# Daniel-Starr/pointcloudhookup

Hardware: AMD Instinct MI355X
Metric: Mpts/s ground-filter+tower-cluster, 100 M-pt corridor; % HBM roofline on kNN (higher is better)
Workload: dtype f32 (filter) + f64 (distance predicate)

## Files before the change

### pointcloudhookup_amd/csrc/pch_dbscan.hip

```cpp
#include "pch_prims.h"

namespace pch {

constexpr int DB_THREADS = 256;
constexpr int DB_WAVES   = DB_THREADS / 64;
constexpr int DB_ROWS    = 25;
constexpr int INT_BIG    = 0x7fffffff;
constexpr int DB_FEW_QUERIES = 24;
constexpr int DB_AHEAD = 3;
constexpr long long DB_LONG_TOT = 8192;
constexpr int DB_SEGS = 43;

struct DbGrid {
    float   ox, oy, oz;
    double  cell;
    double  inv_cell;
    double  eps2;
    float   eps2_lo, eps2_hi;
    int     bx, by, bz;
    int     mx, my, mz;
    int64_t chunk_size;
    const uint32_t* chunk_bad;
    const uint32_t* chunk_cells;
    int     min_samples;
};

__constant__ int8_t DB_ROW_DY[DB_ROWS] = {0, 1, -1, 0, 0, 1, 1, -1, -1, 2, -2, 0, 0,
                                          2, 2, -2, -2, 1, 1, -1, -1, 2, 2, -2, -2};
__constant__ int8_t DB_ROW_DZ[DB_ROWS] = {0, 0, 0, 1, -1, 1, -1, 1, -1, 0, 0, 2, -2,
                                          1, -1, 1, -1, 2, -2, 2, -2, 2, -2, 2, -2};

__device__ __forceinline__ uint64_t db_pack(const DbGrid& g, uint64_t chunk, uint64_t cz,
                                            uint64_t cy, uint64_t cx) {
    return ((((chunk << g.bz) | cz) << g.by | cy) << g.bx) | cx;
}

__device__ __forceinline__ bool db_within(const float4& q, const float4& p, double eps2) {
    const double dx = (double)q.x - (double)p.x;
    const double dy = (double)q.y - (double)p.y;
    const double dz = (double)q.z - (double)p.z;
    double d = dx * dx;
    d += dy * dy;
    d += dz * dz;
    return d <= eps2;
}

__device__ __forceinline__ bool db_within2(const float4& q, const float4& p, const DbGrid& g) {
    const float dx = q.x - p.x, dy = q.y - p.y, dz = q.z - p.z;
    float d = dx * dx;
    d = __builtin_fmaf(dy, dy, d);
    d = __builtin_fmaf(dz, dz, d);
    if (d <= g.eps2_lo) return true;
    if (d >= g.eps2_hi) return false;
    return db_within(q, p, g.eps2);
}

typedef float f32x2 __attribute__((ext_vector_type(2)));
struct __attribute__((aligned(16))) DbPair { f32x2 x, y, z, pad; };

__device__ __forceinline__ void db_tile_put(DbPair* __restrict__ tile, int l, const float4& p) {
    float* f = reinterpret_cast<float*>(&tile[l >> 1]);
    f[l & 1] = p.x; f[2 + (l & 1)] = p.y; f[4 + (l & 1)] = p.z;
}
__device__ __forceinline__ float4 db_tile_get(const DbPair* __restrict__ tile, int k) {
    const float* f = reinterpret_cast<const float*>(&tile[k >> 1]);
    float4 p;
    p.x = f[k & 1]; p.y = f[2 + (k & 1)]; p.z = f[4 + (k & 1)]; p.w = 0.0f;
    return p;
}
__device__ __forceinline__ int db_tile_count(const float4& q, const DbPair* __restrict__ tile, int nj,
                                             const DbGrid& g) {
    const f32x2 qx = {q.x, q.x}, qy = {q.y, q.y}, qz = {q.z, q.z};
    const float lo = g.eps2_lo, hi = g.eps2_hi;
    int c_lo = 0, c_hi = 0;
    const int np = ((nj + 7) & ~7) >> 1;
    for (int k = 0; k < np; k += 4) {
        f32x2 px[4], py[4], pz[4];
#pragma unroll
        for (int u = 0; u < 4; ++u) { px[u] = tile[k + u].x; py[u] = tile[k + u].y; pz[u] = tile[k + u].z; }
#pragma unroll
        for (int u = 0; u < 4; ++u) {
            const f32x2 dx = qx - px[u], dy = qy - py[u], dz = qz - pz[u];
            f32x2 d = dx * dx;
            d = __builtin_elementwise_fma(dy, dy, d);
            d = __builtin_elementwise_fma(dz, dz, d);
            c_lo += (d.x <= lo ? 1 : 0) + (d.y <= lo ? 1 : 0);
            c_hi += (d.x < hi ? 1 : 0) + (d.y < hi ? 1 : 0);
        }
    }
    if (c_lo != c_hi) {
        c_lo = 0;
        for (int k = 0; k < nj; ++k) c_lo += db_within2(q, db_tile_get(tile, k), g) ? 1 : 0;
    }
// ... 638 lines not shown
            cell_key[cc[j]] = key;
            uint4* a4 = reinterpret_cast<uint4*>(cell_acc + 8 * (int64_t)cc[j]);
            a4[0] = make_uint4(0u, 0u, 0u, 0u);
            a4[1] = make_uint4(0u, 0u, 0u, 0u);
            const uint64_t ch = sh < 64 ? key >> sh : 0, pch = sh < 64 ? pk >> sh : 0;
            if (i == 0 || ch != pch) chunk_cells[ch] = cc[j];
        }
        if (i == n - 1) { cell_start[cc[j] + 1] = (uint32_t)n; chunk_cells[nchunks] = cc[j] + 1; }
    }
    if (base + DC_ITEMS <= n) {
        uint4* o = reinterpret_cast<uint4*>(cid + base);
        o[0] = make_uint4(cc[0], cc[1], cc[2], cc[3]);
        o[1] = make_uint4(cc[4], cc[5], cc[6], cc[7]);
    } else {
#pragma unroll
        for (int j = 0; j < DC_ITEMS; ++j)
            if (base + j < n) cid[base + j] = cc[j];
    }
}
struct RowSet {
    int ca[DB_ROWS], cb[DB_ROWS];
};

__device__ __forceinline__ int db_lower(const uint64_t* __restrict__ a, int m, uint64_t k) {
    int lo = 0, hi = m;
    while (lo < hi) { const int mid = (lo + hi) >> 1; if (a[mid] < k) lo = mid + 1; else hi = mid; }
    return lo;
}
__device__ __forceinline__ int2 db_row_run(const DbGrid& g, const uint64_t* __restrict__ cell_key, uint64_t key,
                                           int row) {
    const uint64_t cx = key & ((1ull << g.bx) - 1);
    const uint64_t cy = (key >> g.bx) & ((1ull << g.by) - 1);
    const uint64_t cz = (key >> (g.bx + g.by)) & ((1ull << g.bz) - 1);
    const int sh = g.bx + g.by + g.bz;
    const uint64_t chunk = sh < 64 ? (key >> sh) : 0;
    const int ny = (int)cy + DB_ROW_DY[row], nz = (int)cz + DB_ROW_DZ[row];
    int2 v;
    v.x = 0; v.y = 0;
    if (ny >= 0 && ny <= g.my && nz >= 0 && nz <= g.mz) {
        const int xlo = (int)cx - 2 < 0 ? 0 : (int)cx - 2;
        const int xhi = (int)cx + 2 > g.mx ? g.mx : (int)cx + 2;
        const int c0 = (int)g.chunk_cells[chunk], c1 = (int)g.chunk_cells[chunk + 1];
        v.x = c0 + db_lower(cell_key + c0, c1 - c0, db_pack(g, chunk, (uint64_t)nz, (uint64_t)ny, (uint64_t)xlo));
        const uint64_t khi = db_pack(g, chunk, (uint64_t)nz, (uint64_t)ny, (uint64_t)xhi);
        uint64_t kk[5];
#pragma unroll
        for (int i = 0; i < 5; ++i) kk[i] = v.x + i < c1 ? cell_key[v.x + i] : ~0ull;
        int cntx = 0;
#pragma unroll
        for (int i = 0; i < 5; ++i) cntx += kk[i] <= khi ? 1 : 0;
        v.y = v.x + cntx;
    }
    return v;
}

__device__ __forceinline__ void db_rows(const DbGrid& g, const uint64_t* __restrict__ cell_key, uint64_t key,
                                        RowSet* __restrict__ rs, const int2* __restrict__ rowtab, int cell) {
    const int l = lane_id();
    if (rowtab) {
        if (l < DB_ROWS) {
            const int2 v = rowtab[(int64_t)cell * DB_ROWS + l];
            rs->ca[l] = v.x;
            rs->cb[l] = v.y;
        }
        __builtin_amdgcn_wave_barrier();
        return;
    }
    if (l < DB_ROWS) {
        const int2 v = db_row_run(g, cell_key, key, l);
        rs->ca[l] = v.x;
        rs->cb[l] = v.y;
    }
    __builtin_amdgcn_wave_barrier();
}

__global__ __launch_bounds__(DB_THREADS) void db_rowtab_k(DbGrid g, const uint64_t* __restrict__ cell_key,
                                                          int m, int2* __restrict__ rowtab) {
    const int c = (blockIdx.x * DB_WAVES + wave_id()) * 2 + (lane_id() >> 5);
    const int l = lane_id() & 31;
    if (c >= m || l >= DB_ROWS) return;
    rowtab[(int64_t)c * DB_ROWS + l] = db_row_run(g, cell_key, cell_key[c], l);
}

template <bool COUNT>
__global__ __launch_bounds__(DB_THREADS) void db_core_k(DbGrid g, const float4* __restrict__ pts,
                                                        const uint32_t* __restrict__ cell_start,
                                                        const uint64_t* __restrict__ cell_key, int m,
                                                        const int2* __restrict__ rowtab,
                                                        uint8_t* __restrict__ core_s,
                                                        uint32_t* __restrict__ cell_ncore,
                                                        unsigned long long* __restrict__ stats) {
    unsigned long long n_useful = 0, n_slots = 0, n_tiles = 0;
    auto tally = [&]() {
        if (COUNT && lane_id() == 0) {
            atomicAdd(&stats[0], n_useful); atomicAdd(&stats[1], n_slots);
            atomicAdd(&stats[2], 1ull); atomicAdd(&stats[3], n_tiles);
        }
    };
    __shared__ RowSet rows[DB_WAVES];
    __shared__ DbPair tiles[DB_WAVES][32];
    __shared__ uint32_t seg_a[DB_WAVES][DB_SEGS], seg_b[DB_WAVES][DB_SEGS];
    const int c = blockIdx.x * DB_WAVES + wave_id();
    if (c >= m) return;
    const int l = lane_id();
    const uint32_t s = cell_start[c], e = cell_start[c + 1];
    const int cnt = (int)(e - s);
    {
        const int sh = g.bx + g.by + g.bz;
        if (g.chunk_bad[sh < 64 ? (cell_key[c] >> sh) : 0]) {
            for (uint32_t i = s + l; i < e; i += 64) core_s[i] = 0;
            if (l == 0) cell_ncore[c] = 0;
            return;
        }
    }
    if (cnt >= g.min_samples) {
        for (uint32_t i = s + l; i < e; i += 64) core_s[i] = 1;
        if (l == 0) cell_ncore[c] = (uint32_t)cnt;
        return;
    }
    RowSet* rs = &rows[wave_id()];
    db_rows(g, cell_key, cell_key[c], rs, rowtab, c);
    long long tot = 0;
    if (l < DB_ROWS) tot = (long long)cell_start[rs->cb[l]] - (long long)cell_start[rs->ca[l]];
    tot = wave_reduce_add(tot);
    if (tot < (long long)g.min_samples) {
        for (uint32_t i = s + l; i < e; i += 64) core_s[i] = 0;
        if (l == 0) cell_ncore[c] = 0;
        return;
    }
    uint32_t* sa = seg_a[wave_id()];
    uint32_t* sb = seg_b[wave_id()];
    {
        const uint64_t xmask = (1ull << g.bx) - 1;
        const int cx = (int)(cell_key[c] & xmask);
        if (l < DB_ROWS) {
            const int ca = rs->ca[l], cb = rs->cb[l];
            if (l < 9) {
                int ia = ca, ib = cb;
                if (ca < cb) {
                    if ((int)(cell_key[ca] & xmask) == cx - 2) ia = ca + 1;
                    if (ib > ia && (int)(cell_key[cb - 1] & xmask) == cx + 2) ib = cb - 1;
                }
                sa[l] = cell_start[ia];      sb[l] = cell_start[ib];
                sa[9 + l] = cell_start[ca];  sb[9 + l] = cell_start[ia];
                sa[18 + l] = cell_start[ib]; sb[18 + l] = cell_start[cb];
            } else {
                sa[18 + l] = cell_start[ca]; sb[18 + l] = cell_start[cb];
            }
        }
        __builtin_amdgcn_wave_barrier();
    }
    uint32_t ncore = 0;
    const bool long_sweep = tot >= DB_LONG_TOT;
    if (cnt < DB_FEW_QUERIES) {
        for (uint32_t q = s; q < e; ++q) {
            const float4 qp = pts[q];
            int count = 0;
            if (long_sweep) {
                for (int r = 0; r < DB_SEGS && count < g.min_samples; ++r) {
                    const uint32_t pa = sa[r], pb = sb[r];
                    for (uint32_t j0 = pa; j0 < pb && count < g.min_samples; j0 += 64u * DB_AHEAD) {
                        float4 P[DB_AHEAD];
#pragma unroll
                        for (int u = 0; u < DB_AHEAD; ++u) {
                            const uint32_t j = j0 + 64u * u + l;
                            P[u] = pts[j < pb ? j : pb - 1];
                        }
#pragma unroll
                        for (int u = 0; u < DB_AHEAD; ++u) {
                            const uint32_t jb = j0 + 64u * u;
                            const bool hit = jb + l < pb && db_within2(qp, P[u], g);
                            count += (int)__popcll(__ballot(hit));
                            if (COUNT && jb < pb) { n_useful += (pb - jb) < 64u ? (pb - jb) : 64u; n_slots += 64; }
                        }
                    }
                }
            } else {
                for (int r = 0; r < DB_SEGS && count < g.min_samples; ++r) {
                    const uint32_t pa = sa[r], pb = sb[r];
                    for (uint32_t j0 = pa; j0 < pb && count < g.min_samples; j0 += 64) {
                        const uint32_t j = j0 + l;
                        bool hit = false;
                        if (j < pb) hit = db_within2(qp, pts[j], g);
                        count += (int)__popcll(__ballot(hit));
                        if (COUNT) { n_useful += (pb - j0) < 64u ? (pb - j0) : 64u; n_slots += 64; }
                    }
                }
            }
            const bool is_core = count >= g.min_samples;
            if (l == 0) core_s[q] = is_core ? 1 : 0;
            ncore += is_core;
        }
        if (l == 0) cell_ncore[c] = ncore;
        tally();
        return;
    }
    DbPair* tile = tiles[wave_id()];
    for (uint32_t q0 = s; q0 < e; q0 += 64) {
        const bool valid = q0 + l < e;
        float4 Q;
        Q.x = Q.y = Q.z = 3.0e37f; Q.w = 0.0f;
        if (valid) Q = pts[q0 + l];
        int count = 0;
        unsigned long long active = __ballot(valid);
        int r = 0;
        uint32_t j0 = sa[0];
        while (r < DB_SEGS && __popcll(active) >= DB_FEW_QUERIES / 2) {
            const uint32_t pb = sb[r];
            if (j0 >= pb) { ++r; if (r < DB_SEGS) j0 = sa[r]; continue; }
            const int nj = (int)((pb - j0) < 64u ? (pb - j0) : 64u);
            float4 P;
            P.x = P.y = P.z = 3.0e38f; P.w = 0.0f;
            if (l < nj) P = pts[j0 + l];
            __builtin_amdgcn_wave_barrier();
            db_tile_put(tile, l, P);
            __builtin_amdgcn_wave_barrier();
            count += db_tile_count(Q, tile, nj, g);
            if (COUNT) {
                n_useful += (unsigned long long)__popcll(__ballot(valid)) * (unsigned)nj;
                n_slots += 64ull * (unsigned)((nj + 7) & ~7);
                ++n_tiles;
            }
            j0 += 64;
            active = __ballot(valid && count < g.min_samples);
        }
        while (active) {
            const int ql = (int)__builtin_ctzll(active);
            active &= active - 1;
            float4 qp;
            qp.x = __shfl(Q.x, ql, 64); qp.y = __shfl(Q.y, ql, 64); qp.z = __shfl(Q.z, ql, 64); qp.w = 0.0f;
            int cq = __shfl(count, ql, 64);
            int rr = r;
            uint32_t jj = j0;
            if (long_sweep) {
                while (rr < DB_SEGS && cq < g.min_samples) {
                    const uint32_t pb = sb[rr];
                    if (jj >= pb) { ++rr; if (rr < DB_SEGS) jj = sa[rr]; continue; }
                    float4 P[DB_AHEAD];
#pragma unroll
                    for (int u = 0; u < DB_AHEAD; ++u) {
                        const uint32_t j = jj + 64u * u + l;
                        P[u] = pts[j < pb ? j : pb - 1];
                    }
#pragma unroll
                    for (int u = 0; u < DB_AHEAD; ++u) {
                        const uint32_t jb = jj + 64u * u;
                        const bool hit = jb + l < pb && db_within2(qp, P[u], g);
                        cq += (int)__popcll(__ballot(hit));
                        if (COUNT && jb < pb) { n_useful += (pb - jb) < 64u ? (pb - jb) : 64u; n_slots += 64; }
                    }
                    jj += 64u * DB_AHEAD;
                }
            } else {
                while (rr < DB_SEGS && cq < g.min_samples) {
                    const uint32_t pb = sb[rr];
                    if (jj >= pb) { ++rr; if (rr < DB_SEGS) jj = sa[rr]; continue; }
                    const uint32_t j = jj + l;
                    bool hit = false;
                    if (j < pb) hit = db_within2(qp, pts[j], g);
                    cq += (int)__popcll(__ballot(hit));
                    if (COUNT) { n_useful += (pb - jj) < 64u ? (pb - jj) : 64u; n_slots += 64; }
                    jj += 64;
                }
            }
            if (l == ql) count = cq;
        }
        const bool is_core = valid && count >= g.min_samples;
        if (valid) core_s[q0 + l] = is_core ? 1 : 0;
        ncore += (uint32_t)__popcll(__ballot(is_core));
    }
    if (l == 0) cell_ncore[c] = ncore;
    tally();
}

constexpr int DB_CS_ROUNDS = 16;

__device__ __forceinline__ void db_cellstats_flush(uint32_t* __restrict__ acc, uint32_t c, const uint32_t (&v)[7]) {
#pragma unroll
    for (int k = 0; k < 7; ++k)
        if (v[k]) atomicMax(&acc[8 * (int64_t)c + k], v[k]);
}

__global__ __launch_bounds__(DB_THREADS) void db_cellstats_k(const float4* __restrict__ pts,
                                                             const uint32_t* __restrict__ cid,
                                                             const uint8_t* __restrict__ core_s, int64_t n,
                                                             uint32_t* __restrict__ acc,
                                                             uint32_t* __restrict__ bits, int64_t nw) {
    {
        const int64_t t = (int64_t)blockIdx.x * DB_THREADS + threadIdx.x;
        if (t < nw) bits[t] = 0u;
    }
    const int64_t base = ((int64_t)blockIdx.x * DB_WAVES + wave_id()) * (64 * DB_CS_ROUNDS);
    if (base >= n) return;
    const int l = lane_id();
    constexpr uint32_t NONE = 0xFFFFFFFFu;
    uint32_t carry_c = NONE;
    uint32_t carry[7] = {0, 0, 0, 0, 0, 0, 0};
    uint32_t mine[7] = {0, 0, 0, 0, 0, 0, 0};
    auto fold_mine = [&]() {
#pragma unroll
        for (int k = 0; k < 7; ++k) {
            const uint32_t t = wave_reduce_max(mine[k]);
            carry[k] = t > carry[k] ? t : carry[k];
            mine[k] = 0;
        }
    };
    for (int r0 = 0; r0 < DB_CS_ROUNDS; r0 += 4) {
    if (base + r0 * 64 >= n) break;
    uint32_t c4[4], core4[4];
    float4 p4[4];
#pragma unroll
    for (int u = 0; u < 4; ++u) {
        const int64_t i = base + (r0 + u) * 64 + l;
        const bool in = i < n;
        c4[u] = in ? cid[i] : NONE - 1u;
        core4[u] = in ? core_s[i] : 0u;
        p4[u] = pts[in ? i : base];
    }
#pragma unroll
    for (int u = 0; u < 4; ++u) {
        const int64_t i = base + (r0 + u) * 64 + l;
        const bool in = i < n;
        const uint32_t c = c4[u];
        uint32_t v[7] = {0, 0, 0, 0, 0, 0, 0};
        if (core4[u]) {
            const float4 p = p4[u];
            const uint32_t kx = f32_ordered(p.x), ky = f32_ordered(p.y), kz = f32_ordered(p.z);
            v[0] = ~kx; v[1] = ~ky; v[2] = ~kz; v[3] = kx; v[4] = ky; v[5] = kz;
            v[6] = ~__float_as_uint(p.w);
        }
        if (__ballot(c != carry_c) == 0) {
#pragma unroll
            for (int k = 0; k < 7; ++k) mine[k] = v[k] > mine[k] ? v[k] : mine[k];
            continue;
        }
        if (carry_c != NONE) fold_mine();
#pragma unroll
        for (int o = 1; o < 64; o <<= 1) {
            const uint32_t cu = __shfl_up(c, o, 64);
            const bool same = l >= o && cu == c;
#pragma unroll
            for (int k = 0; k < 7; ++k) {
                const uint32_t t = __shfl_up(v[k], o, 64);
                if (same) v[k] = t > v[k] ? t : v[k];
            }
        }
        const uint32_t c0 = (uint32_t)__builtin_amdgcn_readlane((int)c, 0);
        if (carry_c != NONE) {
            if (carry_c == c0) {
                if (c == c0) {
#pragma unroll
                    for (int k = 0; k < 7; ++k) v[k] = carry[k] > v[k] ? carry[k] : v[k];
                }
            } else if (l == 0) {
                db_cellstats_flush(acc, carry_c, carry);
// ... 671 lines not shown
    }
    best = wave_reduce_min(best);
    if (l == 0 && best != 0xFFFFFFFFu) {
        const int32_t slot = atomicAdd(out_count, 1);
        if (slot < cap) {
            out_pairs[2 * slot] = (int32_t)best;
            out_pairs[2 * slot + 1] = cell_label[c];
        }
    }
}

__global__ void db_prelabel_k(const uint32_t* __restrict__ total, int32_t* __restrict__ out_nclusters,
                              uint32_t* __restrict__ box_acc, int64_t box_words) {
    if (threadIdx.x == 0 && blockIdx.x == 0) *out_nclusters = (int32_t)*total;
    const int64_t i = (int64_t)blockIdx.x * blockDim.x + threadIdx.x;
    if (box_acc && i < box_words) box_acc[i] = 0u;
}

struct DbWs {
    uint32_t* meta;
    uint64_t *k0, *k1, *cell_key;
    uint32_t *v0, *v1, *head, *cid, *cell_start, *cell_ncore, *flag, *radix_ws, *scan_ws;
    float4   *pts, *xbuf;
    uint8_t*  core_s;
    float*    cell_box;
    uint32_t* cell_acc;
    int*      cell_min;
    int      *parent, *root, *comp_min, *cell_label;
    int2*     rowtab;
    int64_t   rowtab_cells;
    uint32_t* chunk_bad;
    uint32_t* chunk_ovf;
    uint32_t* chunk_cells;
    uint32_t* comp;
    uint32_t* flag2;
    unsigned long long* core_stats;
    uint32_t* scan1_b;
};

static void db_plan(Arena& a, int64_t n, DbWs& w) {
    const int64_t nn = n > 0 ? n : 1;
    w.meta = a.take<uint32_t>(64);
    w.scan1_b = a.take<uint32_t>(scan1_ws_u32(nn / 32 + 1));
    w.chunk_cells = a.take<uint32_t>(nn + 8);
    w.core_stats = a.take<unsigned long long>(4);
    w.chunk_bad = a.take<uint32_t>(nn + 8);
    w.chunk_ovf = a.take<uint32_t>(nn + 8);
    w.k0 = a.take<uint64_t>(nn);
    w.k1 = a.take<uint64_t>(nn);
    w.v0 = a.take<uint32_t>(nn);
    w.v1 = a.take<uint32_t>(nn);
    w.head = a.take<uint32_t>(nn + 8);
    w.cid = a.take<uint32_t>(nn);
    w.pts = a.take<float4>(nn);
    w.xbuf = a.take<float4>(nn);
    w.core_s = a.take<uint8_t>(nn);
    w.cell_key = a.take<uint64_t>(nn);
    w.cell_start = a.take<uint32_t>(nn + 8);
    w.cell_ncore = a.take<uint32_t>(nn);
    w.cell_box = a.take<float>(6 * nn);
    w.cell_acc = a.take<uint32_t>(8 * nn);
    w.cell_min = a.take<int>(nn);
    w.parent = a.take<int>(nn);
    w.root = a.take<int>(nn);
    w.comp_min = a.take<int>(nn);
    w.cell_label = a.take<int>(nn);
    w.flag = a.take<uint32_t>(nn / 16 + 256);
    w.radix_ws = a.take<uint32_t>(radix_ws_u32(nn));
    w.scan_ws = a.take<uint32_t>(scan_ws_u32(nn));
    w.rowtab_cells = nn / 4 > 65536 ? nn / 4 : (nn < 65536 ? nn : 65536);
    w.rowtab = a.take<int2>((size_t)w.rowtab_cells * DB_ROWS);
    w.comp = a.take<uint32_t>(3 * nn);
    w.flag2 = a.take<uint32_t>(nn + 8);
}

struct DbCells {
    DbGrid g; const float4* pts; const uint32_t* cell_start; const uint64_t* cell_key; int m;
    const int2* rowtab;
    const uint8_t* core_s; const uint32_t* cell_ncore; const float* cell_box;
};
#define DB_GRID_ARGS(c) (c).g, (c).pts, (c).cell_start, (c).cell_key, (c).m, (c).rowtab
#define DB_CELL_ARGS(c) DB_GRID_ARGS(c), (c).core_s, (c).cell_ncore, (c).cell_box

struct DbTuning { int sort_mode; bool no_boxfold, no_xcd, count_pairs; };
static int g_sort_mode = -1;
static thread_local bool g_count_pairs = false;
static DbTuning db_tuning() {
    static const bool no_boxfold = getenv("PCH_DB_NO_BOXFOLD") != nullptr, no_xcd = getenv("PCH_DB_NO_XCD") != nullptr;
    int m = __atomic_load_n(&g_sort_mode, __ATOMIC_RELAXED);
    if (m < 0) {
        const char* e = getenv("PCH_DBSCAN_SORT");
        m = (e && strcmp(e, "chunk") == 0) ? 1 : (e && strcmp(e, "global") == 0) ? 2 : 0;
        __atomic_store_n(&g_sort_mode, m, __ATOMIC_RELAXED);
    }
    return {m, no_boxfold, no_xcd, g_count_pairs};
}

struct DbLastRun { void* ws; size_t ws_bytes; int64_t n; DbCells c; };
static thread_local DbLastRun g_last = {nullptr, 0, 0, {}};

void ws_touched(const void* base, size_t bytes) {
    if (!g_last.ws) return;
    const char* a0 = static_cast<const char*>(base);
    const char* b0 = static_cast<const char*>(g_last.ws);
    if (a0 < b0 + g_last.ws_bytes && b0 < a0 + bytes) g_last.ws = nullptr;
}

static int db_continue(const char* entry, int64_t n, void* ws, size_t ws_bytes, DbWs& w) {
    if (g_last.ws != ws || g_last.ws_bytes != ws_bytes || g_last.n != n || ws == nullptr) {
        set_error("%s must follow pch_dbscan_f32 of this thread on the same, untouched workspace", entry);
        return PCH_ERR_ARG;
    }
    Arena a(ws, ws_bytes, true);
    db_plan(a, n, w);
    return PCH_OK;
}

static float host_unordered(uint32_t k) {
    uint32_t u = (k & 0x80000000u) ? (k & 0x7fffffffu) : ~k;
    float f;
    memcpy(&f, &u, 4);
    return f;
}

static unsigned db_stride_blocks(int64_t n) { return (unsigned)std::min(ceil_div(n, DB_THREADS * 8), int64_t(2048)); }

struct DbRun {
    const float* xyz; int64_t n, chunk_size, nchunks;
    int32_t* labels; uint8_t* core; int32_t* out_nclusters;
    hipStream_t s; DbWs w;
};

static int db_all_noise(const DbRun& r) {
    PCH_HIP_TRY(hipMemsetAsync(r.labels, 0xFF, sizeof(int32_t) * (size_t)r.n, r.s));
    if (r.core) PCH_HIP_TRY(hipMemsetAsync(r.core, 0, (size_t)r.n, r.s));
    PCH_HIP_TRY(hipMemsetAsync(r.out_nclusters, 0, sizeof(int32_t), r.s));
    return PCH_OK;
}

static int db_bounds(const DbRun& r, const float* aabb_host, float (&box)[6], bool& done) {
    if (aabb_host) {
        memcpy(box, aabb_host, sizeof(box));
    } else {
        uint32_t* meta = r.w.meta;
        PCH_HIP_TRY(hipMemsetAsync(meta, 0xFF, 3 * sizeof(uint32_t), r.s));
        PCH_HIP_TRY(hipMemsetAsync(meta + 3, 0, 3 * sizeof(uint32_t), r.s));
        PCH_LAUNCH("db_aabb_in", db_aabb_in_k, dim3(db_stride_blocks(r.n)), dim3(DB_THREADS), 0, r.s, r.xyz, r.n, meta);
        uint32_t mm[6];
        PCH_HIP_TRY(hipMemcpyAsync(mm, meta, sizeof(mm), hipMemcpyDeviceToHost, r.s));
        PCH_HIP_TRY(hipStreamSynchronize(r.s));
        if (mm[0] == 0xFFFFFFFFu) {
            done = true;
            return db_all_noise(r);
        }
        for (int k = 0; k < 6; ++k) box[k] = host_unordered(mm[k]);
    }
    for (int k = 0; k < 6; ++k) {
        if (!(box[k] == box[k]) || box[k] > 3.0e38f || box[k] < -3.0e38f) {
            set_error("bounding box is not finite");
            return PCH_ERR_ARG;
        }
    }
    return PCH_OK;
}

static int db_cell_bits(DbGrid& g, int mx, int my, int mz) {
    g.mx = mx; g.my = my; g.mz = mz;
    g.bx = bits_for((uint64_t)mx + 1); g.by = bits_for((uint64_t)my + 1); g.bz = bits_for((uint64_t)mz + 1);
    return g.bx + g.by + g.bz;
}

static bool db_grid(const DbRun& r, const float (&box)[6], double eps, int32_t min_samples, DbGrid& g, int& cellbits,
                    int& nbits) {
    g.ox = box[0]; g.oy = box[1]; g.oz = box[2];
    g.cell = eps / 1.7320508075688772 * (1.0 - 1.0 / 65536.0);
    g.inv_cell = 1.0 / g.cell;
    g.eps2 = eps * eps;
    g.eps2_lo = nextafterf((float)(g.eps2 * (1.0 - 1.0 / 1048576.0)), -INFINITY);
// ... 40 lines not shown
    int64_t* first_bad = reinterpret_cast<int64_t*>(w.meta + 12);
    PCH_HIP_TRY(hipMemsetAsync(first_bad, 0xFF, sizeof(int64_t), s));
    PCH_LAUNCH("db_first_bad", db_first_bad_k, dim3(db_stride_blocks(n)), dim3(DB_THREADS), 0, s, r.xyz, n,
               reinterpret_cast<unsigned long long*>(first_bad));
    PCH_HIP_TRY(hipMemsetAsync(w.meta + 6, 0, 6 * sizeof(uint32_t), s));
    for (int axis = 0; axis < 3; ++axis) {
        PCH_LAUNCH("dbc_axis_keys", dbc_axis_keys_k, dim3(gn), dim3(DB_THREADS), 0, s, r.xyz, n, axis, w.k0, w.v0);
        PCH_TRY(radix_sort_pairs(w.k0, w.v0, w.k1, w.v1, n, 32, w.radix_ws, s));
        const bool in1 = radix_sort_result_buffer(32) == 1;
        const uint64_t* ksa = in1 ? w.k1 : w.k0;
        const uint32_t* vsa = in1 ? w.v1 : w.v0;
        PCH_LAUNCH("dbc_heads", dbc_heads_k, dim3(gn), dim3(DB_THREADS), 0, s, ksa, n, g.inv_cell, w.flag2);
        PCH_TRY(scan_exclusive_u32(w.flag2, w.head, n, w.scan_ws, nullptr, s));
        PCH_HIP_TRY(hipMemsetAsync(w.cell_start, 0, sizeof(uint32_t) * (size_t)(n + 8), s));
        for (int phase = 0; phase < 2; ++phase)
            PCH_LAUNCH("dbc_local", dbc_local_k, dim3(gn), dim3(DB_THREADS), 0, s, ksa, w.flag2, w.head, n, g.inv_cell,
                       w.cell_box, phase, w.cid, w.cell_start, w.meta + 6);
        PCH_TRY(scan_exclusive_u32(w.cell_start, w.cell_start, n, w.scan_ws, nullptr, s));
        PCH_LAUNCH("dbc_comp", dbc_comp_k, dim3(gn), dim3(DB_THREADS), 0, s, vsa, w.flag2, w.head, w.cid, w.cell_start,
                   n, axis, w.comp, w.meta + 9);
    }
    uint32_t back[8];
    PCH_HIP_TRY(hipMemcpyAsync(back, w.meta + 6, sizeof(back), hipMemcpyDeviceToHost, s));
    PCH_HIP_TRY(hipStreamSynchronize(s));
    int64_t bad_row;
    memcpy(&bad_row, &back[6], sizeof(bad_row));
    if (bad_row >= 0) {
        PCH_TRY(db_all_noise(r));
        g_last.ws = nullptr;
        done = true;
        return PCH_OK;
    }
    if (back[0] != 0) { set_error("compressed cell coordinates out of range"); return PCH_ERR_RANGE; }
    cellbits = db_cell_bits(g, (int)back[3], (int)back[4], (int)back[5]);
    if (cellbits > 64) {
        set_error("cell key needs %d bits even with compressed coordinates (%lld isolated points?)", cellbits, (long long)n);
        return PCH_ERR_RANGE;
    }
    return PCH_OK;
}

static int db_sorted_keys(const DbRun& r, const DbGrid& g, int cellbits, int nbits, bool compressed, int sort_mode,
                          const uint64_t*& ks) {
    const DbWs& w = r.w; const hipStream_t s = r.s; const int64_t n = r.n, nchunks = r.nchunks;
    const unsigned gn = (unsigned)ceil_div(n, DB_THREADS);
    const size_t bytes = (size_t)(reinterpret_cast<char*>(w.chunk_cells + nchunks + 1) - reinterpret_cast<char*>(w.meta + 4));
    PCH_HIP_TRY(hipMemsetAsync(w.meta + 4, 0, (bytes + 15) & ~size_t(15), s));
    if (!compressed && cellbits <= 31 && r.chunk_size <= CS_MAX_CHUNK && sort_mode != 2 &&
        (sort_mode == 1 || nchunks >= CS_MIN_CHUNKS)) {
        PCH_LAUNCH("db_cellscatter", db_cellscatter_k, dim3((unsigned)nchunks), dim3(CS_THREADS), 0, s, r.xyz, n, g,
                   w.chunk_bad, w.chunk_ovf, w.pts, w.k1, w.meta + 6);
        PCH_LAUNCH("db_chunksort", db_chunksort_k, dim3((unsigned)nchunks), dim3(CS_THREADS), 0, s, r.xyz, n, g,
                   w.chunk_ovf, w.chunk_bad, w.xbuf, w.pts, w.k1, w.meta + 6, (unsigned long long*)w.cell_box);
#ifdef PCH_CS_STAMPS
        {
            unsigned long long t[11];
            PCH_HIP_TRY(hipStreamSynchronize(s));
            PCH_HIP_TRY(hipMemcpy(t, w.cell_box, sizeof(t), hipMemcpyDeviceToHost));
            for (int q = 1; q <= 6; ++q)
                fprintf(stderr, "chunksort phase %d: %.2f us\n", q, (double)(long long)(t[q] - t[q - 1]) / 100.0);
            fprintf(stderr, "chunksort tiles: rank %.2f us, offsets %.2f us, scatter %.2f us\n", (double)t[8] / 100.0,
                    (double)t[9] / 100.0, (double)t[10] / 100.0);
        }
#endif
        ks = w.k1;
        return PCH_OK;
    }
    PCH_HIP_TRY(hipMemsetAsync(w.chunk_bad, 0, sizeof(uint32_t) * (size_t)(nchunks + 1), s));
    if (compressed) {
        PCH_LAUNCH("db_keys_comp", db_keys_comp_k, dim3(gn), dim3(DB_THREADS), 0, s, w.comp, n, g, w.k0, w.v0);
    } else {
        PCH_LAUNCH("db_chunkbad", db_chunkbad_k, dim3(db_stride_blocks(n)), dim3(DB_THREADS), 0, s, r.xyz, n,
                   r.chunk_size, w.chunk_bad);
        PCH_LAUNCH("db_keys", db_keys_k, dim3(gn), dim3(DB_THREADS), 0, s, r.xyz, n, g, w.chunk_bad, w.k0, w.v0,
                   w.meta + 6);
    }
    PCH_TRY(radix_sort_pairs(w.k0, w.v0, w.k1, w.v1, n, nbits, w.radix_ws, s));
    const bool in1 = radix_sort_result_buffer(nbits) == 1;
    ks = in1 ? w.k1 : w.k0;
    PCH_LAUNCH("db_gather", db_gather_k, dim3(gn), dim3(DB_THREADS), 0, s, r.xyz, ks, in1 ? w.v1 : w.v0, n, w.pts);
    return PCH_OK;
}

static int db_cells_core(const DbRun& r, const DbGrid& g, int cellbits, const uint64_t* ks, bool count_pairs,
                         DbCells& c) {
    const DbWs& w = r.w; const hipStream_t s = r.s; const int64_t n = r.n;
    const int64_t ntile = ceil_div(n, (int64_t)SCAN_TILE);
    PCH_LAUNCH("db_heads", db_heads_k, dim3((unsigned)ntile), dim3(DB_THREADS), 0, s, ks, n, w.scan_ws);
    PCH_TRY(scan_tile_sums_u32(w.scan_ws, ntile, w.meta + 7, s));
    uint32_t st_m[2];
    PCH_TRY(peek_enqueue(w.meta + 6, sizeof(st_m), s));
    PCH_LAUNCH("db_cells", db_cells_k, dim3((unsigned)ntile), dim3(DB_THREADS), 0, s, ks, w.scan_ws, n, cellbits,
               r.nchunks, w.cid, w.cell_start, w.cell_key, w.chunk_cells, w.cell_acc);
    PCH_TRY(peek_wait(st_m, sizeof(st_m)));
    if (st_m[0] != 0) {
        set_error("finite coordinates outside the supplied bounding box");
        return PCH_ERR_ARG;
    }
    const int m = (int)st_m[1];
    const unsigned gc = (unsigned)ceil_div(m, DB_WAVES);
    c = {g, w.pts, w.cell_start, w.cell_key, m, m <= w.rowtab_cells ? w.rowtab : nullptr, w.core_s, w.cell_ncore,
         w.cell_box};
    if (c.rowtab)
        PCH_LAUNCH("db_rowtab", db_rowtab_k, dim3((unsigned)ceil_div(m, 2 * DB_WAVES)), dim3(DB_THREADS), 0, s, g,
                   w.cell_key, m, w.rowtab);
    if (count_pairs) {
        PCH_HIP_TRY(hipMemsetAsync(w.core_stats, 0, 4 * sizeof(unsigned long long), s));
        PCH_LAUNCH("db_core_counting", db_core_k<true>, dim3(gc), dim3(DB_THREADS), 0, s, DB_GRID_ARGS(c), w.core_s,
                   w.cell_ncore, w.core_stats);
    } else {
        PCH_LAUNCH("db_core", db_core_k<false>, dim3(gc), dim3(DB_THREADS), 0, s, DB_GRID_ARGS(c), w.core_s,
                   w.cell_ncore, nullptr);
    }
    PCH_LAUNCH("db_cellstats", db_cellstats_k, dim3((unsigned)ceil_div(n, (int64_t)DB_WAVES * 64 * DB_CS_ROUNDS)),
               dim3(DB_THREADS), 0, s, w.pts, w.cid, w.core_s, n, w.cell_acc, w.flag, ceil_div(n, 32));
    PCH_LAUNCH("db_cellfin", db_cellfin_k, dim3((unsigned)ceil_div(m, DB_THREADS)), dim3(DB_THREADS), 0, s,
               w.cell_acc, m, w.cell_box, w.cell_min, w.parent, w.comp_min);
    return PCH_OK;
}

static int db_union(const DbRun& r, const DbCells& c) {
    const DbWs& w = r.w; const hipStream_t s = r.s; const int m = c.m;
    const unsigned gc = (unsigned)ceil_div(m, DB_WAVES);
    const uint8_t* face_todo = nullptr;
    if (c.rowtab) {
        PCH_LAUNCH("db_union_pairs", db_union_pairs_k, dim3((unsigned)ceil_div(4 * (int64_t)m, DB_THREADS)),
                   dim3(DB_THREADS), 0, s, DB_CELL_ARGS(c), w.parent, reinterpret_cast<uint8_t*>(w.root));
        face_todo = reinterpret_cast<const uint8_t*>(w.root);
    }
    PCH_LAUNCH("db_union0", db_union_face_k, dim3(gc), dim3(DB_THREADS), 0, s, DB_CELL_ARGS(c), w.parent, face_todo);
    PCH_LAUNCH("db_flatten", db_flatten_k, dim3((unsigned)ceil_div(m, DB_THREADS)), dim3(DB_THREADS), 0, s,
               w.parent, m);
    PCH_LAUNCH("db_union1", db_union_k, dim3(gc), dim3(DB_THREADS), 0, s, DB_CELL_ARGS(c), w.parent);
    PCH_LAUNCH("db_compmin", db_compmin_k, dim3((unsigned)ceil_div(m, DB_THREADS)), dim3(DB_THREADS), 0, s,
               w.cell_min, w.cell_ncore, m, w.parent, w.root, w.comp_min);
    return PCH_OK;
}

static int db_labels(const DbRun& r, const DbCells& c, const DbTuning& tune, int32_t* k_host, DbBoxOut* boxes) {
    const DbWs& w = r.w; const hipStream_t s = r.s; const int64_t n = r.n, nchunks = r.nchunks; const int m = c.m;
    const int64_t nw = ceil_div(n, 32);
    uint32_t* bits = w.flag;
    uint32_t* wrank = w.flag + ((nw + 63) & ~int64_t(63));
    static_assert(DB_CS_ROUNDS * 64 * DB_WAVES / DB_THREADS <= 32, "db_cellstats_k's grid has a thread per bitmap word");
    PCH_LAUNCH("db_mark", db_mark_k, dim3((unsigned)ceil_div(m, DB_THREADS)), dim3(DB_THREADS), 0, s,
               w.root, w.comp_min, m, bits);
    if (scan1_pays(nw)) PCH_TRY(scan1_exclusive_popc_u32(bits, wrank, nw, w.scan1_b, w.meta + 8, s));
    else PCH_TRY(scan_exclusive_popc_u32(bits, wrank, nw, w.scan_ws, w.meta + 8, s));
    uint32_t* box_acc = (boxes && boxes->acc && boxes->cap > 0 && !tune.no_boxfold) ? boxes->acc : nullptr;
    const int32_t box_cap = box_acc ? boxes->cap : 0;
    PCH_LAUNCH("db_prelabel", db_prelabel_k, dim3((unsigned)(box_acc ? ceil_div(8 * (int64_t)box_cap, 256) : 1)),
               dim3(256), 0, s, w.meta + 8, r.out_nclusters, box_acc, 8 * (int64_t)box_cap);
    if (k_host) PCH_TRY(peek_enqueue(r.out_nclusters, sizeof(int32_t), s));
    const int bpc = (nchunks >= 16 && !tune.no_xcd) ? (int)ceil_div(r.chunk_size, DB_LAB_TILE) : 0;
    const unsigned gl = bpc > 0 ? (unsigned)(8 * ceil_div(nchunks, 8) * bpc) : (unsigned)ceil_div(n, DB_LAB_TILE);
    PCH_LAUNCH("db_label", db_label_k, dim3(gl), dim3(DB_THREADS), 0, s, w.pts, w.cid, w.core_s, w.root, w.comp_min,
               bits, wrank, n, w.cell_start, w.cell_label, r.labels, r.core, r.chunk_size, bpc, nchunks, box_acc,
               box_cap);
    PCH_LAUNCH("db_border", db_border_k, dim3((unsigned)ceil_div(m, DB_WAVES)), dim3(DB_THREADS), 0, s,
               DB_CELL_ARGS(c), w.cell_label, r.labels, box_acc, box_cap);
    if (box_acc) boxes->done = true;
    if (k_host) {
        PCH_TRY(peek_wait(k_host, sizeof(int32_t)));
        if (*k_host < 0) {
            set_error("stage C: a device-side look-back wait ran out of its budget; outputs are undefined");
            return PCH_ERR_TIMEOUT;
        }
    }
    return PCH_OK;
}

}

using namespace pch;

extern "C" int pch_first_nonfinite_row_f32(const float* xyz, int64_t n, int64_t* out_row, void* stream) {
    PCH_DEVICE_GUARD(out_row);
    hipStream_t s = (hipStream_t)stream;
    PCH_REQUIRE(n >= 0 && out_row && (n == 0 || xyz), "bad argument");
    PCH_HIP_TRY(hipMemsetAsync(out_row, 0xFF, sizeof(int64_t), s));
    if (n == 0) return PCH_OK;
    PCH_LAUNCH("db_first_bad", db_first_bad_k, dim3(db_stride_blocks(n)), dim3(DB_THREADS), 0, s, xyz, n,
               reinterpret_cast<unsigned long long*>(out_row));
    return PCH_OK;
}

extern "C" void pch_dbscan_set_sort_mode(int mode) {
    __atomic_store_n(&g_sort_mode, (mode == 1 || mode == 2) ? mode : 0, __ATOMIC_RELAXED);
}

extern "C" size_t pch_dbscan_ws_bytes(int64_t n) {
    if (n < 0) return 0;
    Arena a;
    DbWs w;
    db_plan(a, n, w);
    return a.off;
}

int pch::dbscan_run(const float* xyz, int64_t n, double eps, int32_t min_samples, int64_t chunk_size,
                    const float* aabb_host, int32_t* labels, uint8_t* core, int32_t* out_nclusters, void* ws,
                    size_t ws_bytes, hipStream_t s, int32_t* k_host, DbBoxOut* boxes) {
    if (k_host) *k_host = 0;
    if (boxes) boxes->done = false;
    PCH_REQUIRE(n >= 0 && n < (int64_t(1) << 31), "n out of range [0, 2^31)");
    PCH_REQUIRE(eps > 0.0, "eps must be > 0 (sklearn: InvalidParameterError)");
    PCH_REQUIRE(min_samples >= 1, "min_samples must be >= 1 (sklearn: InvalidParameterError)");
    PCH_REQUIRE(out_nclusters != nullptr, "out_nclusters is null");
    if (n == 0) {
        PCH_HIP_TRY(hipMemsetAsync(out_nclusters, 0, sizeof(int32_t), s));
        return PCH_OK;
    }
    PCH_REQUIRE(xyz && labels && ws, "null buffer");
    Arena a(ws, ws_bytes);
    DbWs w;
    db_plan(a, n, w);
    if (a.overflow) { set_error("workspace too small: need %zu bytes", a.off); return PCH_ERR_WORKSPACE; }
    if (chunk_size <= 0 || chunk_size > n) chunk_size = n;
    const DbRun r = {xyz, n, chunk_size, ceil_div(n, chunk_size), labels, core, out_nclusters, s, w};
    const DbTuning tune = db_tuning();

    float box[6];
    bool done = false;
    PCH_TRY(db_bounds(r, aabb_host, box, done));
    if (done) return PCH_OK;
    DbGrid g;
    int cellbits, nbits;
    const bool overflow = db_grid(r, box, eps, min_samples, g, cellbits, nbits);
    if (overflow) {
        if (r.nchunks > 1) return db_run_chunks(r, eps, min_samples, ws, ws_bytes, k_host);
        PCH_TRY(db_compress(r, g, cellbits, done));
        if (done) return PCH_OK;
        nbits = cellbits;
    }
    const uint64_t* ks;
    DbCells c;
    PCH_TRY(db_sorted_keys(r, g, cellbits, nbits, overflow, tune.sort_mode, ks));
    PCH_TRY(db_cells_core(r, g, cellbits, ks, tune.count_pairs, c));
    PCH_TRY(db_union(r, c));
    PCH_TRY(db_labels(r, c, tune, k_host, boxes));
    g_last = {ws, ws_bytes, n, c};
    return PCH_OK;
}

extern "C" int pch_dbscan_first_core_rows_i32(int64_t n, int32_t* out_rows, void* ws, size_t ws_bytes, void* stream) {
    PCH_DEVICE_GUARD(out_rows ? (const void*)out_rows : (const void*)ws);
    PCH_REQUIRE(n >= 0, "bad argument");
    if (n == 0) return PCH_OK;
    DbWs w;
    PCH_TRY(db_continue(__func__, n, ws, ws_bytes, w));
    PCH_REQUIRE(out_rows != nullptr, "null output");
    const int64_t nw = ceil_div(n, 32);
    const uint32_t* bits = w.flag;
    const uint32_t* wrank = w.flag + ((nw + 63) & ~int64_t(63));
    PCH_LAUNCH("db_first_rows", db_first_rows_k, dim3((unsigned)ceil_div(nw, DB_THREADS)), dim3(DB_THREADS), 0,
               (hipStream_t)stream, bits, wrank, nw, out_rows);
    return PCH_OK;
}

extern "C" void pch_dbscan_set_pair_counting(int enable) { g_count_pairs = enable != 0; }

extern "C" int pch_dbscan_pair_stats(int64_t n, uint64_t* out4_host, void* ws, size_t ws_bytes, void* stream) {
    PCH_DEVICE_GUARD(ws);
    PCH_REQUIRE(n >= 0 && out4_host, "bad argument");
    memset(out4_host, 0, 4 * sizeof(uint64_t));
    if (n == 0) return PCH_OK;
    DbWs w;
    PCH_TRY(db_continue(__func__, n, ws, ws_bytes, w));
    PCH_HIP_TRY(hipMemcpyAsync(out4_host, w.core_stats, 4 * sizeof(uint64_t), hipMemcpyDeviceToHost, (hipStream_t)stream));
    PCH_HIP_TRY(hipStreamSynchronize((hipStream_t)stream));
    return PCH_OK;
}

extern "C" int pch_dbscan_strip_pairs_i32(int64_t n, float x_lo, float x_hi, int32_t cap, int32_t* out_pairs,
                                          int32_t* out_count, void* ws, size_t ws_bytes, void* stream) {
    PCH_DEVICE_GUARD(out_count);
    hipStream_t s = (hipStream_t)stream;
    PCH_REQUIRE(n >= 0 && cap >= 0 && out_count && (cap == 0 || out_pairs), "bad argument");
    PCH_HIP_TRY(hipMemsetAsync(out_count, 0, sizeof(int32_t), s));
    if (n == 0 || !(x_lo < x_hi)) return PCH_OK;
    DbWs w;
    PCH_TRY(db_continue(__func__, n, ws, ws_bytes, w));
    const int m = g_last.c.m;
    PCH_LAUNCH("db_strip_pairs", db_strip_pairs_k, dim3((unsigned)ceil_div(m, DB_WAVES)), dim3(DB_THREADS), 0, s,
               w.pts, w.cell_start, w.core_s, w.cell_ncore, w.cell_box, w.cell_label, m, x_lo, x_hi, cap, out_pairs,
               out_count);
    return PCH_OK;
}

extern "C" int pch_dbscan_relabel_i32(const int32_t* map, int32_t nmap, int64_t n, int32_t* labels, void* ws,
                                      size_t ws_bytes, void* stream) {
    PCH_DEVICE_GUARD(labels);
    hipStream_t s = (hipStream_t)stream;
    PCH_REQUIRE(n >= 0 && nmap >= 0 && (nmap == 0 || map) && (n == 0 || labels), "bad argument");
    if (n == 0) return PCH_OK;
    DbWs w;
    PCH_TRY(db_continue(__func__, n, ws, ws_bytes, w));
    const DbCells& c = g_last.c;
    PCH_LAUNCH("db_remap_points", db_remap_points_k, dim3((unsigned)ceil_div(n, DB_THREADS)), dim3(DB_THREADS), 0, s,
               w.pts, w.core_s, n, map, nmap, labels);
    PCH_LAUNCH("db_remap_cells", db_remap_cells_k, dim3((unsigned)ceil_div(c.m, DB_THREADS)), dim3(DB_THREADS), 0, s,
               w.cell_label, w.cell_ncore, c.m, map, nmap);
    PCH_LAUNCH("db_border", db_border_k, dim3((unsigned)ceil_div(c.m, DB_WAVES)), dim3(DB_THREADS), 0, s,
               DB_CELL_ARGS(c), w.cell_label, labels, nullptr, 0);
    return PCH_OK;
}

extern "C" int pch_dbscan_f32(const float* xyz, int64_t n, double eps, int32_t min_samples,
                              int64_t chunk_size, const float* aabb_host, int32_t* labels,
                              uint8_t* core, int32_t* out_nclusters, void* ws, size_t ws_bytes,
                              void* stream) {
    PCH_DEVICE_GUARD(xyz ? (const void*)xyz : (const void*)out_nclusters);
    return dbscan_run(xyz, n, eps, min_samples, chunk_size, aabb_host, labels, core, out_nclusters, ws, ws_bytes,
                      (hipStream_t)stream, nullptr);
}
```

Baseline: 61470.

## Split long-sweep DBSCAN core cells into deferred per-query work items

Cells whose neighborhood sweep is long are no longer handled by a single wave in db_core_k. They are appended to a list and processed in a second kernel that scans a limited number of tiles per query. Queries still undecided after that are emitted as work items, and a third kernel splits each item's remaining neighbor range into 32 parts, accumulating hit counts atomically. The aim is to remove load imbalance from dense cells that serialize on one wave. The cost is extra launches, atomics and list writes into the reused xbuf scratch, plus relying on meta counters being zeroed, which the diff does not visibly do.

```diff
diff --git a/pointcloudhookup_amd/csrc/pch_dbscan.hip b/pointcloudhookup_amd/csrc/pch_dbscan.hip
--- a/pointcloudhookup_amd/csrc/pch_dbscan.hip
+++ b/pointcloudhookup_amd/csrc/pch_dbscan.hip
@@ -9,6 +9,11 @@
 constexpr int DB_FEW_QUERIES = 24;
 constexpr int DB_AHEAD = 3;
 constexpr long long DB_LONG_TOT = 8192;
+constexpr int DB_SPLIT_TILES = 8;
+constexpr int DB_ITEM_PARTS = 32;
+constexpr int DB_PART_GROUPS = 8;
+constexpr uint32_t DB_PART = 64u * DB_PART_GROUPS;
+constexpr int DB_LONG_BLOCKS = 1024;
 constexpr int DB_SEGS = 43;
 
 struct DbGrid {
@@ -813,14 +818,46 @@
     rowtab[(int64_t)c * DB_ROWS + l] = db_row_run(g, cell_key, cell_key[c], l);
 }
 
-template <bool COUNT>
-__global__ __launch_bounds__(DB_THREADS) void db_core_k(DbGrid g, const float4* __restrict__ pts,
-                                                        const uint32_t* __restrict__ cell_start,
-                                                        const uint64_t* __restrict__ cell_key, int m,
-                                                        const int2* __restrict__ rowtab,
-                                                        uint8_t* __restrict__ core_s,
-                                                        uint32_t* __restrict__ cell_ncore,
-                                                        unsigned long long* __restrict__ stats) {
+__device__ __forceinline__ void db_segments(const DbGrid& g, const uint32_t* __restrict__ cell_start,
+                                            const uint64_t* __restrict__ cell_key, int c,
+                                            const RowSet* __restrict__ rs, uint32_t* __restrict__ sa,
+                                            uint32_t* __restrict__ sb) {
+    const int l = lane_id();
+    const uint64_t xmask = (1ull << g.bx) - 1;
+    const int cx = (int)(cell_key[c] & xmask);
+    if (l < DB_ROWS) {
+        const int ca = rs->ca[l], cb = rs->cb[l];
+        if (l < 9) {
+            int ia = ca, ib = cb;
+            if (ca < cb) {
+                if ((int)(cell_key[ca] & xmask) == cx - 2) ia = ca + 1;
+                if (ib > ia && (int)(cell_key[cb - 1] & xmask) == cx + 2) ib = cb - 1;
+            }
+            sa[l] = cell_start[ia];      sb[l] = cell_start[ib];
+            sa[9 + l] = cell_start[ca];  sb[9 + l] = cell_start[ia];
+            sa[18 + l] = cell_start[ib]; sb[18 + l] = cell_start[cb];
+        } else {
+            sa[18 + l] = cell_start[ca]; sb[18 + l] = cell_start[cb];
+        }
+    }
+    __builtin_amdgcn_wave_barrier();
+}
+
+struct DbSplit {
+    uint32_t* qcount;
+    uint32_t* cells;
+    uint2* items;
+    uint32_t* ncells;
+    uint32_t* nitems;
+};
+
+template <bool COUNT, bool SPLIT>
+__device__ __forceinline__ void db_core_cell(const DbGrid& g, const float4* __restrict__ pts,
+                                             const uint32_t* __restrict__ cell_start,
+                                             const uint64_t* __restrict__ cell_key, const int2* __restrict__ rowtab,
+                                             uint8_t* __restrict__ core_s, uint32_t* __restrict__ cell_ncore,
+                                             const DbSplit& sp, unsigned long long* __restrict__ stats, int c,
+                                             RowSet* rs, DbPair* tile, uint32_t* sa, uint32_t* sb) {
     unsigned long long n_useful = 0, n_slots = 0, n_tiles = 0;
     auto tally = [&]() {
         if (COUNT && lane_id() == 0) {
@@ -828,11 +865,6 @@
             atomicAdd(&stats[2], 1ull); atomicAdd(&stats[3], n_tiles);
         }
     };
-    __shared__ RowSet rows[DB_WAVES];
-    __shared__ DbPair tiles[DB_WAVES][32];
-    __shared__ uint32_t seg_a[DB_WAVES][DB_SEGS], seg_b[DB_WAVES][DB_SEGS];
-    const int c = blockIdx.x * DB_WAVES + wave_id();
-    if (c >= m) return;
     const int l = lane_id();
     const uint32_t s = cell_start[c], e = cell_start[c + 1];
     const int cnt = (int)(e - s);
@@ -849,7 +881,6 @@
         if (l == 0) cell_ncore[c] = (uint32_t)cnt;
         return;
     }
-    RowSet* rs = &rows[wave_id()];
     db_rows(g, cell_key, cell_key[c], rs, rowtab, c);
     long long tot = 0;
     if (l < DB_ROWS) tot = (long long)cell_start[rs->cb[l]] - (long long)cell_start[rs->ca[l]];
@@ -859,31 +890,15 @@
         if (l == 0) cell_ncore[c] = 0;
         return;
     }
-    uint32_t* sa = seg_a[wave_id()];
-    uint32_t* sb = seg_b[wave_id()];
-    {
-        const uint64_t xmask = (1ull << g.bx) - 1;
-        const int cx = (int)(cell_key[c] & xmask);
-        if (l < DB_ROWS) {
-            const int ca = rs->ca[l], cb = rs->cb[l];
-            if (l < 9) {
-                int ia = ca, ib = cb;
-                if (ca < cb) {
-                    if ((int)(cell_key[ca] & xmask) == cx - 2) ia = ca + 1;
-                    if (ib > ia && (int)(cell_key[cb - 1] & xmask) == cx + 2) ib = cb - 1;
-                }
-                sa[l] = cell_start[ia];      sb[l] = cell_start[ib];
-                sa[9 + l] = cell_start[ca];  sb[9 + l] = cell_start[ia];
-                sa[18 + l] = cell_start[ib]; sb[18 + l] = cell_start[cb];
-            } else {
-                sa[18 + l] = cell_start[ca]; sb[18 + l] = cell_start[cb];
-            }
-        }
-        __builtin_amdgcn_wave_barrier();
-    }
+    const bool long_sweep = tot >= DB_LONG_TOT;
+    if (!SPLIT && long_sweep && sp.cells) {
+        if (l == 0) sp.cells[atomicAdd(sp.ncells, 1u)] = (uint32_t)c;
+        return;
+    }
+    db_segments(g, cell_start, cell_key, c, rs, sa, sb);
     uint32_t ncore = 0;
-    const bool long_sweep = tot >= DB_LONG_TOT;
-    if (cnt < DB_FEW_QUERIES) {
+    const bool split = SPLIT;
+    if (cnt < DB_FEW_QUERIES && !split) {
         for (uint32_t q = s; q < e; ++q) {
             const float4 qp = pts[q];
             int count = 0;
@@ -926,7 +941,6 @@
         tally();
         return;
     }
-    DbPair* tile = tiles[wave_id()];
     for (uint32_t q0 = s; q0 < e; q0 += 64) {
         const bool valid = q0 + l < e;
         float4 Q;
@@ -936,7 +950,9 @@
         unsigned long long active = __ballot(valid);
         int r = 0;
         uint32_t j0 = sa[0];
-        while (r < DB_SEGS && __popcll(active) >= DB_FEW_QUERIES / 2) {
+        int tiles = 0;
+        uint32_t passed = 0;
+        while (r < DB_SEGS && (__popcll(active) >= DB_FEW_QUERIES / 2 || (split && active && tiles < DB_SPLIT_TILES))) {
             const uint32_t pb = sb[r];
             if (j0 >= pb) { ++r; if (r < DB_SEGS) j0 = sa[r]; continue; }
             const int nj = (int)((pb - j0) < 64u ? (pb - j0) : 64u);
@@ -953,8 +969,12 @@
                 ++n_tiles;
             }
             j0 += 64;
+            ++tiles;
+            passed += (uint32_t)nj;
             active = __ballot(valid && count < g.min_samples);
         }
+        const unsigned long long deferred = (split && r < DB_SEGS) ? active : 0ull;
+        active &= ~deferred;
         while (active) {
             const int ql = (int)__builtin_ctzll(active);
             active &= active - 1;
@@ -999,9 +1019,116 @@
         const bool is_core = valid && count >= g.min_samples;
         if (valid) core_s[q0 + l] = is_core ? 1 : 0;
         ncore += (uint32_t)__popcll(__ballot(is_core));
+        if (SPLIT && ((deferred >> l) & 1ull)) {
+            sp.items[atomicAdd(sp.nitems, 1u)] = make_uint2(q0 + (uint32_t)l, passed);
+            sp.qcount[q0 + l] = (uint32_t)count;
+        }
     }
     if (l == 0) cell_ncore[c] = ncore;
     tally();
+}
+
+template <bool COUNT>
+__global__ __launch_bounds__(DB_THREADS) void db_core_k(DbGrid g, const float4* __restrict__ pts,
+                                                        const uint32_t* __restrict__ cell_start,
+                                                        const uint64_t* __restrict__ cell_key, int m,
+                                                        const int2* __restrict__ rowtab,
+                                                        uint8_t* __restrict__ core_s,
+                                                        uint32_t* __restrict__ cell_ncore,
+                                                        DbSplit sp,
+                                                        unsigned long long* __restrict__ stats) {
+    __shared__ RowSet rows[DB_WAVES];
+    __shared__ DbPair tiles[DB_WAVES][32];
+    __shared__ uint32_t seg_a[DB_WAVES][DB_SEGS], seg_b[DB_WAVES][DB_SEGS];
+    const int c = blockIdx.x * DB_WAVES + wave_id();
+    if (c >= m) return;
+    db_core_cell<COUNT, false>(g, pts, cell_start, cell_key, rowtab, core_s, cell_ncore, sp, stats, c,
+                               &rows[wave_id()], tiles[wave_id()], seg_a[wave_id()], seg_b[wave_id()]);
+}
+
+template <bool COUNT>
+__global__ __launch_bounds__(DB_THREADS) void db_core_cells_k(DbGrid g, const float4* __restrict__ pts,
+                                                              const uint32_t* __restrict__ cell_start,
+                                                              const uint64_t* __restrict__ cell_key, int m,
+                                                              const int2* __restrict__ rowtab,
+                                                              uint8_t* __restrict__ core_s,
+                                                              uint32_t* __restrict__ cell_ncore,
+                                                              DbSplit sp,
+                                                              unsigned long long* __restrict__ stats) {
+    __shared__ RowSet rows[DB_WAVES];
+    __shared__ DbPair tiles[DB_WAVES][32];
+    __shared__ uint32_t seg_a[DB_WAVES][DB_SEGS], seg_b[DB_WAVES][DB_SEGS];
+    const uint32_t nc = *sp.ncells;
+    for (uint32_t i = blockIdx.x * DB_WAVES + wave_id(); i < nc; i += gridDim.x * DB_WAVES)
+        db_core_cell<COUNT, true>(g, pts, cell_start, cell_key, rowtab, core_s, cell_ncore, sp, stats,
+                                  (int)sp.cells[i], &rows[wave_id()], tiles[wave_id()], seg_a[wave_id()],
+                                  seg_b[wave_id()]);
+}
+
+template <bool COUNT>
+__global__ __launch_bounds__(DB_THREADS) void db_core_long_k(DbGrid g, const float4* __restrict__ pts,
+                                                             const uint32_t* __restrict__ cell_start,
+                                                             const uint64_t* __restrict__ cell_key, int m,
+                                                             const int2* __restrict__ rowtab,
+                                                             const uint32_t* __restrict__ cid, DbSplit sp,
+                                                             uint8_t* __restrict__ core_s,
+                                                             uint32_t* __restrict__ cell_ncore,
+                                                             unsigned long long* __restrict__ stats) {
+    const uint64_t np = (uint64_t)*sp.nitems * DB_ITEM_PARTS;
+    const int l = lane_id();
+    const uint32_t ms = (uint32_t)g.min_samples;
+    __shared__ RowSet rows[DB_WAVES];
+    __shared__ uint32_t seg_a[DB_WAVES][DB_SEGS], seg_b[DB_WAVES][DB_SEGS];
+    RowSet* rs = &rows[wave_id()];
+    uint32_t* sa = seg_a[wave_id()];
+    uint32_t* sb = seg_b[wave_id()];
+    unsigned long long n_useful = 0, n_slots = 0;
+    for (uint64_t p = (uint64_t)blockIdx.x * DB_WAVES + wave_id(); p < np; p += (uint64_t)gridDim.x * DB_WAVES) {
+        const uint32_t item = (uint32_t)(p / DB_ITEM_PARTS), k = (uint32_t)(p % DB_ITEM_PARTS);
+        const uint2 qf = sp.items[item];
+        const uint32_t have = __hip_atomic_load(&sp.qcount[qf.x], __ATOMIC_RELAXED, __HIP_MEMORY_SCOPE_AGENT);
+        const float4 qp = pts[qf.x];
+        const int c = (int)cid[qf.x];
+        if (have >= ms) continue;
+        db_rows(g, cell_key, cell_key[c], rs, rowtab, c);
+        db_segments(g, cell_start, cell_key, c, rs, sa, sb);
+        const uint2 v = l < DB_SEGS ? make_uint2(sa[l], sb[l]) : make_uint2(0u, 0u);
+        const uint32_t len = v.y - v.x;
+        const uint32_t incl = wave_scan_incl(len);
+        const uint32_t base = v.x - (incl - len);
+        const uint32_t tot = __shfl(incl, 63, 64), rem = tot - qf.y;
+        const uint32_t ps = (rem + DB_ITEM_PARTS - 1) / DB_ITEM_PARTS;
+        const uint32_t f0 = qf.y + k * ps, f1 = f0 + ps < tot ? f0 + ps : tot;
+        if (f0 >= f1) continue;
+        uint32_t hits = 0;
+        for (uint32_t fb = f0; fb < f1; fb += DB_PART) {
+            float4 P[DB_PART_GROUPS];
+#pragma unroll
+            for (int u = 0; u < DB_PART_GROUPS; ++u) {
+                const uint32_t f = fb + 64u * u + l < f1 ? fb + 64u * u + l : f1 - 1;
+                int sg = 0;
+#pragma unroll
+                for (int b = 32; b > 0; b >>= 1)
+                    if (__shfl(incl, sg + b - 1, 64) <= f) sg += b;
+                P[u] = pts[__shfl(base, sg, 64) + f];
+            }
+#pragma unroll
+            for (int u = 0; u < DB_PART_GROUPS; ++u) {
+                const uint32_t fg = fb + 64u * u;
+                const bool hit = fg + l < f1 && db_within2(qp, P[u], g);
+                hits += (uint32_t)__popcll(__ballot(hit));
+                if (COUNT && fg < f1) { n_useful += (f1 - fg) < 64u ? (f1 - fg) : 64u; n_slots += 64; }
+            }
+        }
+        if (l == 0 && hits > 0) {
+            const uint32_t old = atomicAdd(&sp.qcount[qf.x], hits);
+            if (old < ms && old + hits >= ms) {
+                core_s[qf.x] = 1;
+                atomicAdd(&cell_ncore[c], 1u);
+            }
+        }
+    }
+    if (COUNT && l == 0 && n_slots) { atomicAdd(&stats[0], n_useful); atomicAdd(&stats[1], n_slots); }
 }
 
 constexpr int DB_CS_ROUNDS = 16;
@@ -1839,18 +1966,19 @@
 #define DB_GRID_ARGS(c) (c).g, (c).pts, (c).cell_start, (c).cell_key, (c).m, (c).rowtab
 #define DB_CELL_ARGS(c) DB_GRID_ARGS(c), (c).core_s, (c).cell_ncore, (c).cell_box
 
-struct DbTuning { int sort_mode; bool no_boxfold, no_xcd, count_pairs; };
+struct DbTuning { int sort_mode; bool no_boxfold, no_xcd, no_split, count_pairs; };
 static int g_sort_mode = -1;
 static thread_local bool g_count_pairs = false;
 static DbTuning db_tuning() {
-    static const bool no_boxfold = getenv("PCH_DB_NO_BOXFOLD") != nullptr, no_xcd = getenv("PCH_DB_NO_XCD") != nullptr;
+    static const bool no_boxfold = getenv("PCH_DB_NO_BOXFOLD") != nullptr, no_xcd = getenv("PCH_DB_NO_XCD") != nullptr,
+                      no_split = getenv("PCH_DB_NO_SPLIT") != nullptr;
     int m = __atomic_load_n(&g_sort_mode, __ATOMIC_RELAXED);
     if (m < 0) {
         const char* e = getenv("PCH_DBSCAN_SORT");
         m = (e && strcmp(e, "chunk") == 0) ? 1 : (e && strcmp(e, "global") == 0) ? 2 : 0;
         __atomic_store_n(&g_sort_mode, m, __ATOMIC_RELAXED);
     }
-    return {m, no_boxfold, no_xcd, g_count_pairs};
+    return {m, no_boxfold, no_xcd, no_split, g_count_pairs};
 }
 
 struct DbLastRun { void* ws; size_t ws_bytes; int64_t n; DbCells c; };
@@ -2057,7 +2185,7 @@
     return PCH_OK;
 }
 
-static int db_cells_core(const DbRun& r, const DbGrid& g, int cellbits, const uint64_t* ks, bool count_pairs,
+static int db_cells_core(const DbRun& r, const DbGrid& g, int cellbits, const uint64_t* ks, const DbTuning& tune,
                          DbCells& c) {
     const DbWs& w = r.w; const hipStream_t s = r.s; const int64_t n = r.n;
     const int64_t ntile = ceil_div(n, (int64_t)SCAN_TILE);
@@ -2079,13 +2207,35 @@
     if (c.rowtab)
         PCH_LAUNCH("db_rowtab", db_rowtab_k, dim3((unsigned)ceil_div(m, 2 * DB_WAVES)), dim3(DB_THREADS), 0, s, g,
                    w.cell_key, m, w.rowtab);
-    if (count_pairs) {
+    DbSplit sp = {nullptr, nullptr, nullptr, nullptr, nullptr};
+    if (!tune.no_split) {
+        static_assert(2 * sizeof(uint32_t) + sizeof(uint2) == sizeof(float4), "the lists fill w.xbuf");
+        sp.qcount = reinterpret_cast<uint32_t*>(w.xbuf);
+        sp.cells = sp.qcount + n;
+        sp.items = reinterpret_cast<uint2*>(sp.cells + n);
+        sp.ncells = w.meta + 16;
+        sp.nitems = w.meta + 17;
+    }
+    const unsigned gl = (unsigned)std::max<int64_t>(1, std::min<int64_t>(DB_LONG_BLOCKS, ceil_div(n, DB_WAVES)));
+    if (tune.count_pairs) {
         PCH_HIP_TRY(hipMemsetAsync(w.core_stats, 0, 4 * sizeof(unsigned long long), s));
         PCH_LAUNCH("db_core_counting", db_core_k<true>, dim3(gc), dim3(DB_THREADS), 0, s, DB_GRID_ARGS(c), w.core_s,
-                   w.cell_ncore, w.core_stats);
+                   w.cell_ncore, sp, w.core_stats);
+        if (sp.cells) {
+            PCH_LAUNCH("db_core_cells_counting", db_core_cells_k<true>, dim3(gl), dim3(DB_THREADS), 0, s,
+                       DB_GRID_ARGS(c), w.core_s, w.cell_ncore, sp, w.core_stats);
+            PCH_LAUNCH("db_core_long_counting", db_core_long_k<true>, dim3(gl), dim3(DB_THREADS), 0, s, DB_GRID_ARGS(c),
+                       w.cid, sp, w.core_s, w.cell_ncore, w.core_stats);
+        }
     } else {
         PCH_LAUNCH("db_core", db_core_k<false>, dim3(gc), dim3(DB_THREADS), 0, s, DB_GRID_ARGS(c), w.core_s,
-                   w.cell_ncore, nullptr);
+                   w.cell_ncore, sp, nullptr);
+        if (sp.cells) {
+            PCH_LAUNCH("db_core_cells", db_core_cells_k<false>, dim3(gl), dim3(DB_THREADS), 0, s, DB_GRID_ARGS(c),
+                       w.core_s, w.cell_ncore, sp, nullptr);
+            PCH_LAUNCH("db_core_long", db_core_long_k<false>, dim3(gl), dim3(DB_THREADS), 0, s, DB_GRID_ARGS(c), w.cid,
+                       sp, w.core_s, w.cell_ncore, nullptr);
+        }
     }
     PCH_LAUNCH("db_cellstats", db_cellstats_k, dim3((unsigned)ceil_div(n, (int64_t)DB_WAVES * 64 * DB_CS_ROUNDS)),
                dim3(DB_THREADS), 0, s, w.pts, w.cid, w.core_s, n, w.cell_acc, w.flag, ceil_div(n, 32));
@@ -2210,7 +2360,7 @@
     const uint64_t* ks;
     DbCells c;
     PCH_TRY(db_sorted_keys(r, g, cellbits, nbits, overflow, tune.sort_mode, ks));
-    PCH_TRY(db_cells_core(r, g, cellbits, ks, tune.count_pairs, c));
+    PCH_TRY(db_cells_core(r, g, cellbits, ks, tune, c));
     PCH_TRY(db_union(r, c));
     PCH_TRY(db_labels(r, c, tune, k_host, boxes));
     g_last = {ws, ws_bytes, n, c};
```

Result: slower. 53770, median of 2 (-12.5%).
